# apache/parquet-mr

Measured on AMD Instinct MI355X. Metric: decoded values/s, device-resident int64 RLE_DICTIONARY pages, higher is better.
Workload: dtype int64; 1 GPU; C2: int64 RLE_DICTIONARY, 1k-cardinality dictionary (w=10), Zipf(a=1.5) run lengths in [1,4096], parquet-mr V1 pages of 20,000 values, uncompressed, one 100M-row row group per GPU; rows_per_gpu=100000000, pages_per_gpu=5000, encoded_data_bytes_per_gpu=4368634, parallelism=row-group shard x1

## Files before the change

### include/pqgpu.h

```cpp
#ifndef PQGPU_H
#define PQGPU_H

#include <stddef.h>
#include <stdint.h>

#ifdef __cplusplus
extern "C" {
#endif

#define PQG_ABI_VERSION 6

enum pqg_physical_type {
  PQG_BOOLEAN = 0,
  PQG_INT32 = 1,
  PQG_INT64 = 2,
  PQG_INT96 = 3,
  PQG_FLOAT = 4,
  PQG_DOUBLE = 5,
  PQG_BYTE_ARRAY = 6,
  PQG_FIXED_LEN_BYTE_ARRAY = 7
};

enum pqg_encoding {
  PQG_PLAIN = 0,
// ... 76 lines not shown
  int64_t value_index;
  char message[240];
} pqg_status;

typedef struct pqg_ctx pqg_ctx;
typedef struct pqg_plan pqg_plan;


int pqg_abi_version(void);

int pqg_device_count(void);

int pqg_ctx_create(int device, void* hip_stream, pqg_ctx** out);
int pqg_ctx_destroy(pqg_ctx* ctx);
void* pqg_ctx_stream(pqg_ctx* ctx);

enum pqg_dispatch {
  PQG_DISPATCH_PLAIN_ONE_PASS = 1,
  PQG_DISPATCH_DICT_DIRECT = 2,
  PQG_DISPATCH_GZIP_PREPASS_MIN = 3,
  PQG_DISPATCH_DICT_FUSED = 4,
  PQG_DISPATCH_NULL_HINTS = 5,
  PQG_DISPATCH_TAKE_STAGED = 6,
  PQG_DISPATCH_ZSTD_PREPASS = 7
};
int pqg_ctx_set_dispatch(pqg_ctx* ctx, int key, int value);

int pqg_decode(pqg_ctx* ctx, const uint8_t* d_bytes, uint64_t n_bytes,
               pqg_column_desc* cols, int n_cols,
               const pqg_page_desc* pages, int n_pages,
               uint32_t* d_page_value_counts, pqg_status* st);

int pqg_sync(pqg_ctx* ctx, pqg_status* st);

enum pqg_phase {
  PQG_PHASE_NONE = 0,
  PQG_PHASE_DICTIONARY = 1,
  PQG_PHASE_RL_INIT = 2,
  PQG_PHASE_DL_INIT = 3,
  PQG_PHASE_DATA_INIT = 4,
  PQG_PHASE_RL_READ = 5,
  PQG_PHASE_DL_READ = 6,
  PQG_PHASE_VALUE = 7
};

typedef struct pqg_page_error {
  int32_t code;
// ... 321 lines not shown
```

### parquet-mr_amd/csrc/pqgpu_api.hip

```cpp
#include <hip/hip_runtime.h>

#include <algorithm>
#include <chrono>
#include <cstdio>
#include <cstddef>
#include <cstdlib>
#include <cstring>
#include <new>
#include <atomic>
#include <thread>
#include <type_traits>
#include <vector>

#include "pqgpu_internal.h"
#include "pqgpu_filter.h"
#include "pqgpu_take.h"

using pqg::ColumnDev;
using pqg::PageWork;
using pqg::HostErr;
using pqg::bin_out;
using pqg::elem_width;
using pqg::out_width;
using pqg::C_DICT4; using pqg::C_DICT8; using pqg::C_IDS; using pqg::C_PLAIN; using pqg::C_BOOL; using pqg::C_DELTA4;
// ... 73 lines not shown
  bool zero;
};

template <class T>
PlanBufInit uploaded(PlanBuf b, const std::vector<T>& v, size_t min_elems) {
  return PlanBufInit{b, v.data(), sizeof(T) * v.size(), sizeof(T) * std::max(v.size(), min_elems), false};
}

}

struct pqg_plan {
  pqg_ctx* ctx = nullptr;
  const uint8_t* d_bytes = nullptr;
  uint64_t n_bytes = 0;
  pqg::PlanLayout L;
  DevBuf buf[B_COUNT];
  uint32_t* dba_meta() const {
    return L.dba_meta_off == pqg::NO_REGION ? nullptr : (uint32_t*)((uint8_t*)buf[B_BSCRATCH].p + L.dba_meta_off);
  }
  uint32_t epoch = 0;
  uint32_t err_epoch = pqg::ERR_EPOCH_MAX;
  uint32_t pseg_epoch = 0;
  bool dict_fused = true;
  bool plain_fused = false;
  bool seg_walk = true;
  bool null_hints = false;
  int kernels = 0;
  int timeout_fallbacks = 0;
  int plain_fallbacks = 0;
  int hint_fallbacks = 0;
  uint32_t* d_counts = nullptr;
  std::vector<pqg_page_error> page_errs;
};

struct RouterCache {
  int w = -1;
  uint64_t tail_len = 0;
  std::vector<uint8_t> bytes;
  std::vector<uint64_t> off;
  std::vector<uint32_t> cnt;
  std::vector<uint64_t> vo;
  std::vector<int32_t> vals;
  uint64_t hits = 0, misses = 0;
};

struct pqg_ctx {
// ... 6 lines not shown
  std::vector<pqg_staged_output> staged;
  pqg_column_desc* last_cols = nullptr;
  PinnedBuf pin_in, pin_out, pin_err;
  DevBuf host_bytes, host_out, host_counts, host_runs;
  DevBuf asm_scratch;
  hipStream_t copy_stream = nullptr;
  DevBuf zstd_scratch;
  DevBuf zstd_seqs, zstd_mode;
  DevBuf gzip_recs, gzip_mode;
  hipStream_t side_stream = nullptr;
  hipEvent_t ev_fork = nullptr, ev_join = nullptr;
  hipStream_t bin_stream = nullptr;
  hipEvent_t ev_join_bin = nullptr;
  hipStream_t fix_stream = nullptr;
  hipEvent_t ev_join_fix = nullptr;
  hipStream_t dent_stream = nullptr;
  hipEvent_t ev_dent_fork = nullptr, ev_dent = nullptr;
  int plain_mode = 2;
  bool dict_direct = true;
  bool dict_fused = true;
  bool null_hints = true;
  uint32_t gz_prepass_min = pqg::GZ_PREPASS_MIN;
  bool zstd_prepass = true;
  RouterCache router;
  DevBuf filter_scratch, filter_image;
  uint64_t filter_serial = 0;
  DevBuf filter_dict;
  PinnedBuf filter_dict_pin;
  hipEvent_t filter_dict_ev[4] = {};
  uint32_t filter_dict_seq = 0;
  pqg_column_desc dict_desc = {};
  pqg_column_desc* dict_user = nullptr;
  static constexpr int TAKE_SLOTS = 4;
  static constexpr size_t TAKE_SLOT_BYTES = sizeof(pqg::TakeRecDev) * pqg::TAKE_REC_MAX_RECORDS;
  DevBuf take_scratch, take_cols;
  PinnedBuf take_pin;
  hipEvent_t take_ev[TAKE_SLOTS] = {};
  uint32_t take_seq = 0;
  bool take_staged = true;
};

extern "C" {

int pqg_abi_version(void) { return PQG_ABI_VERSION; }

const char* pqg_error_name(int code) {
// ... 13 lines not shown
    case PQG_ERR_NO_DICTIONARY: return "NO_DICTIONARY";
    case PQG_ERR_DICT_ENCODING: return "DICT_ENCODING";
    case PQG_ERR_CRC: return "CRC";
    default: return "UNKNOWN";
  }
}

int pqg_device_count(void) {
  int n = 0;
  if (hipGetDeviceCount(&n) != hipSuccess) return 0;
  return n;
}

int pqg_ctx_create(int device, void* hip_stream, pqg_ctx** out) {
  if (!out) return PQG_ERR_INVALID_ARG;
  *out = nullptr;
  int n = pqg_device_count();
  if (n <= 0) return PQG_ERR_NO_DEVICE;
  if (device < 0 || device >= n) return PQG_ERR_INVALID_ARG;
  if (hipSetDevice(device) != hipSuccess) return PQG_ERR_HIP;
  pqg_ctx* c = new (std::nothrow) pqg_ctx();
  if (!c) return PQG_ERR_INVALID_ARG;
  c->device = device;
  if (hip_stream) {
    c->stream = (hipStream_t)hip_stream;
  } else {
    if (hipStreamCreateWithFlags(&c->stream, hipStreamNonBlocking) != hipSuccess) {
      delete c;
      return PQG_ERR_HIP;
    }
    c->own_stream = true;
  }
  if (hipStreamCreateWithFlags(&c->side_stream, hipStreamNonBlocking) != hipSuccess) c->side_stream = nullptr;
  if (hipStreamCreateWithFlags(&c->bin_stream, hipStreamNonBlocking) != hipSuccess) c->bin_stream = nullptr;
  if (hipStreamCreateWithFlags(&c->fix_stream, hipStreamNonBlocking) != hipSuccess) c->fix_stream = nullptr;
  *out = c;
  return PQG_OK;
}

void* pqg_ctx_stream(pqg_ctx* ctx) { return ctx ? (void*)ctx->stream : nullptr; }

int pqg_ctx_set_dispatch(pqg_ctx* ctx, int key, int value) {
  if (!ctx) return PQG_ERR_INVALID_ARG;
  switch (key) {
    case PQG_DISPATCH_PLAIN_ONE_PASS:
      if (value < 0 || value > 3) return PQG_ERR_INVALID_ARG;
// ... 2 lines not shown
    case PQG_DISPATCH_DICT_DIRECT:
      if (value != 0 && value != 1) return PQG_ERR_INVALID_ARG;
      ctx->dict_direct = value != 0;
      return PQG_OK;
    case PQG_DISPATCH_GZIP_PREPASS_MIN:
      if (value < 0) return PQG_ERR_INVALID_ARG;
      ctx->gz_prepass_min = (uint32_t)value;
      return PQG_OK;
    case PQG_DISPATCH_DICT_FUSED:
      if (value != 0 && value != 1) return PQG_ERR_INVALID_ARG;
      ctx->dict_fused = value != 0;
      return PQG_OK;
    case PQG_DISPATCH_NULL_HINTS:
      if (value != 0 && value != 1) return PQG_ERR_INVALID_ARG;
      ctx->null_hints = value != 0;
      return PQG_OK;
    case PQG_DISPATCH_TAKE_STAGED:
      if (value != 0 && value != 1) return PQG_ERR_INVALID_ARG;
      ctx->take_staged = value != 0;
      return PQG_OK;
    case PQG_DISPATCH_ZSTD_PREPASS:
      if (value != 0 && value != 1) return PQG_ERR_INVALID_ARG;
      ctx->zstd_prepass = value != 0;
      return PQG_OK;
    default: return PQG_ERR_INVALID_ARG;
  }
}

int pqg_plan_destroy(pqg_plan* p);

int pqg_ctx_destroy(pqg_ctx* c) {
  if (!c) return PQG_OK;
  (void)hipSetDevice(c->device);
  (void)hipStreamSynchronize(c->stream);
  if (c->last) pqg_plan_destroy(c->last);
  c->pin_in.release();
  c->pin_out.release();
  c->pin_err.release();
  c->host_bytes.release();
  c->host_out.release();
  c->host_counts.release();
  c->host_runs.release();
  c->asm_scratch.release();
  c->zstd_scratch.release();
  c->zstd_seqs.release();
  c->zstd_mode.release();
// ... 49 lines not shown
                            const pqg_column_desc* cols, int n_cols, const pqg_page_desc* pages, int n_pages,
                            pqg_plan** out, pqg_status* st) {
  if (st) { std::memset(st, 0, sizeof(*st)); st->page = -1; }
  if (!ctx || !out || n_cols < 0 || n_pages < 0 || (n_cols && !cols) || (n_pages && !pages) || (n_bytes && !d_bytes) ||
      ((uintptr_t)d_bytes & 3u)) {
    set_status(st, PQG_ERR_INVALID_ARG, -1, -1, "plan arguments");
    return PQG_ERR_INVALID_ARG;
  }
  if (hipSetDevice(ctx->device) != hipSuccess) return PQG_ERR_HIP;
  pqg_plan* P = new (std::nothrow) pqg_plan();
  if (!P) return PQG_ERR_INVALID_ARG;
  P->ctx = ctx;
  P->d_bytes = d_bytes;
  P->n_bytes = n_bytes;
  pqg::PlanLayout& L = P->L;
  int bad_page = -1;
  if (pqg::plan_layout(n_bytes, valid_bytes, cols, n_cols, pages, n_pages,
                       pqg::PlanOptions{ctx->plain_mode, ctx->dict_direct, ctx->null_hints}, &L, &bad_page) != PQG_OK) {
    set_status(st, PQG_ERR_INVALID_ARG, bad_page, -1, "page descriptor");
    delete P;
    return PQG_ERR_INVALID_ARG;
  }
  P->dict_fused = ctx->dict_fused;
  P->plain_fused = L.n_pcp != 0;
  P->null_hints = L.null_hints;
  const size_t pages1 = (size_t)std::max(n_pages, 1);
  const PlanBufInit init[B_COUNT] = {
      uploaded(B_WORK, L.h_work, 0),
      uploaded(B_COLS, L.cols, 0),
      uploaded(B_LISTS, L.flat, 1),
      uploaded(B_COL_PAGES, L.cp, 1),
      uploaded(B_COL_PAGE_START, L.cps, 0),
      {B_ERR, nullptr, 0, err_region_bytes(n_pages, n_cols) + 16, false},
      {B_BSCRATCH, nullptr, 0, (size_t)std::max<uint64_t>(L.scratch_bytes, 256), false},
      uploaded(B_BIN_LISTS, L.bl, 1),
      uploaded(B_BIN_BLOCKS, L.bin_blocks, 1),
      uploaded(B_BIN_CHUNKS, L.bin_chunks, 1),
      uploaded(B_DBA_CHUNKS, L.dba_chunks, 1),
      uploaded(B_SEGS, L.segs, 1),
      uploaded(B_DENT_TILES, L.dent_tiles, 1),
      uploaded(B_PSEGS, L.psegs, 1),
      {B_PSTATUS, nullptr, 2 * sizeof(uint64_t) * L.psegs.size(), 2 * sizeof(uint64_t) * std::max<size_t>(L.psegs.size(), 1), true},
      uploaded(B_PCOL_PAGES, L.pcp, 1),
      {B_PCOL_START, L.pcs.data(), L.pcp.empty() ? 0 : sizeof(int32_t) * L.pcs.size(), sizeof(int32_t) * L.pcs.size(), false},
      {B_REC, nullptr, 0, sizeof(uint64_t) * (size_t)(L.rec_total + 2 * 64 + 16), false},
      {B_CHUNK_RUN, nullptr, 0, sizeof(uint32_t) * std::max<uint32_t>(L.chunk_total, 1), false},
// ... 138 lines not shown
                           (uint32_t*)((uint8_t*)P->buf[B_BSCRATCH].p + P->L.hint_off));
  if (e == hipSuccess && pf) {
    uint8_t* scb = (uint8_t*)P->buf[B_BSCRATCH].p;
    uint64_t* ps = (uint64_t*)P->buf[B_PSTATUS].p;
    e = pqg::launch_bin_plain(fork ? ctx->side_stream : s, P->d_bytes, P->n_bytes, work, cols, (const int32_t*)P->buf[B_PCOL_PAGES].p,
                              (const int32_t*)P->buf[B_PCOL_START].p, P->L.n_pcols, (const uint64_t*)P->buf[B_PSEGS].p, P->L.n_psegs, ps,
                              ps + P->L.n_psegs, (uint32_t*)(scb + P->L.pticket_off), P->pseg_epoch,
                              (uint32_t*)(scb + P->L.pflag_off), P->err_epoch, err, ecount, P->L.plain_pg, P->L.n_pcp);
    if (fork && hipEventRecord(ctx->ev_join, ctx->side_stream) != hipSuccess) e = hipErrorUnknown;
  }
  const hipStream_t sb = fork_bin ? ctx->bin_stream : s;
  const hipStream_t sf = fork_fix ? ctx->fix_stream : s;
  if (e == hipSuccess) e = launch_dict_walks(sb);
  for (int k = 0; k < C_NCLS && e == hipSuccess; k++) {
    int n = P->L.cls_n[k] - (k == C_BINP ? P->L.n_binp_seg + (pf ? P->L.n_binp_fused : 0) : 0);
    if (!n) continue;
    const int32_t* l = lists + P->L.cls_off[k];
    switch (k) {
      case C_DICT4:
      case C_DICT8: {
        const int i = k - C_DICT4;
        e = pqg::launch_dict(k == C_DICT8 ? 8 : 4, sf, P->d_bytes, P->n_bytes, work, cols, l, n, (uint64_t*)P->buf[B_REC].p,
                             (uint32_t*)P->buf[B_CHUNK_RUN].p, (const uint64_t*)P->buf[B_CHUNKS].p + P->L.chunk_off[i], P->L.chunk_n[i],
                             (uint64_t*)P->buf[B_PSTAT].p, (uint32_t*)P->buf[B_FLAGS].p, P->epoch, P->dict_fused, err, ecount);
        break;
      }
      case C_IDS: {
        const int i = k - C_DICT4;
        e = pqg::launch_dict_ids(sb, P->d_bytes, P->n_bytes, work, cols, l, n, (uint64_t*)P->buf[B_REC].p,
                                 (uint32_t*)P->buf[B_CHUNK_RUN].p, (const uint64_t*)P->buf[B_CHUNKS].p + P->L.chunk_off[i],
                                 P->L.chunk_n[i], (uint64_t*)P->buf[B_PSTAT].p, (uint32_t*)P->buf[B_FLAGS].p, P->epoch, P->dict_fused, err, ecount);
        break;
      }
      case C_DD:
      case C_DDG: {
        const int g = k == C_DDG ? 1 : 0;
        e = pqg::launch_dict_dd(sb, P->d_bytes, P->n_bytes, work, cols, l, n, (uint64_t*)P->buf[B_REC].p,
                                (uint32_t*)P->buf[B_CHUNK_RUN].p, (const uint64_t*)P->buf[B_CHUNKS].p + P->L.dd_chunk_off[g],
                                P->L.dd_chunk_n[g], (uint64_t*)P->buf[B_PSTAT].p, (uint32_t*)P->buf[B_FLAGS].p, P->epoch, P->dict_fused,
                                err, ecount, (uint64_t*)((uint8_t*)P->buf[B_BSCRATCH].p + P->L.dd_sums_off[g]),
                                bl + P->L.off_dd_cols[g], bl + P->L.off_dd_start[g], P->L.n_dd_cols[g], P->L.dd_region, g == 1,
                                g == 1 && dent_fork ? ctx->ev_dent : nullptr);
        break;
      }
      case C_BSS: e = pqg::launch_bss(sf, P->d_bytes, P->n_bytes, work, cols, l, n, err, ecount); break;
      case C_BINP:
        e = pqg::launch_bin_walk(sb, P->d_bytes, P->n_bytes, work, cols, l, n, 0, P->L.n_pages, err, ecount);
        break;
      case C_DLBA: e = pqg::launch_dlba_lengths(sb, P->d_bytes, P->n_bytes, work, cols, l, n, err, ecount); break;
      case C_DBA:
        e = pqg::launch_dba_lengths(sb, P->d_bytes, P->n_bytes, work, cols, l, n, err, ecount, P->dba_meta());
        break;
      case C_PLAIN: e = pqg::launch_plain(0, sf, P->d_bytes, P->n_bytes, work, cols, l, n, err, ecount); break;
      case C_BOOL: e = pqg::launch_plain(1, sf, P->d_bytes, P->n_bytes, work, cols, l, n, err, ecount); break;
      case C_RLEBOOL: e = pqg::launch_plain(2, sf, P->d_bytes, P->n_bytes, work, cols, l, n, err, ecount); break;
      case C_DELTA4: e = pqg::launch_delta(4, sf, P->d_bytes, P->n_bytes, work, cols, l, n, err, ecount); break;
      case C_DELTA8: e = pqg::launch_delta(8, sf, P->d_bytes, P->n_bytes, work, cols, l, n, err, ecount); break;
    }
  }
  if (e == hipSuccess && P->L.n_segs && !P->seg_walk)
    e = pqg::launch_bin_walk(sb, P->d_bytes, P->n_bytes, work, cols,
                             lists + P->L.cls_off[C_BINP] + (P->L.cls_n[C_BINP] - P->L.n_binp_seg), P->L.n_binp_seg, 0,
                             P->L.n_pages, err, ecount);
// ... 1369 lines not shown
```

### parquet-mr_amd/csrc/pqgpu_internal.h

```cpp
#pragma once
#include <hip/hip_runtime.h>
#include <stdint.h>

#include "../../include/pqgpu.h"
#include "pqgpu_filter.h"
#include "pqgpu_plan.h"

namespace pqg {

struct ErrCount {
  uint32_t* p;
  uint32_t epoch;
};
constexpr uint32_t ERR_EPOCH_MAX = 0xFFFFu;
constexpr uint64_t ERR_KEY_MASK = (1ull << 48) - 1;

hipError_t launch_dict(int width, hipStream_t st, const uint8_t* bytes, uint64_t n_bytes, PageWork* work,
                       const ColumnDev* cols, const int32_t* list, int n, uint64_t* rec, uint32_t* chunk_run,
                       const uint64_t* chunks, uint32_t n_chunks, uint64_t* pstat, uint32_t* flags, uint32_t epoch,
                       bool fused, uint64_t* err,
                       ErrCount err_count);
hipError_t launch_levels(hipStream_t st, const uint8_t* bytes, uint64_t n_bytes, PageWork* work, const ColumnDev* cols,
                         const int32_t* list, int n, uint64_t* err, ErrCount err_count, uint32_t* hint_bad);
hipError_t launch_scan(hipStream_t st, PageWork* work, const int32_t* col_pages, const int32_t* col_page_start,
                       int n_cols);
hipError_t launch_plain(int kind, hipStream_t st, const uint8_t* bytes, uint64_t n_bytes, PageWork* work,
                        const ColumnDev* cols, const int32_t* list, int n, uint64_t* err, ErrCount err_count);
hipError_t launch_delta(int width, hipStream_t st, const uint8_t* bytes, uint64_t n_bytes, PageWork* work,
                        const ColumnDev* cols, const int32_t* list, int n, uint64_t* err, ErrCount err_count);
hipError_t launch_dict_ids(hipStream_t st, const uint8_t* bytes, uint64_t n_bytes, PageWork* work,
                           const ColumnDev* cols, const int32_t* list, int n, uint64_t* rec, uint32_t* chunk_run,
                           const uint64_t* chunks, uint32_t n_chunks, uint64_t* pstat, uint32_t* flags,
                           uint32_t epoch, bool fused,
                           uint64_t* err, ErrCount err_count);
hipError_t launch_dict_dd(hipStream_t st, const uint8_t* bytes, uint64_t n_bytes, PageWork* work,
                          const ColumnDev* cols, const int32_t* list, int n, uint64_t* rec, uint32_t* chunk_run,
                          const uint64_t* chunks, uint32_t n_chunks, uint64_t* pstat, uint32_t* flags,
                          uint32_t epoch, bool fused, uint64_t* err, ErrCount err_count, uint64_t* sums,
                          const int32_t* dd_cols, const int32_t* dd_start, int n_dd_cols, uint32_t dd_region,
                          bool global, hipEvent_t entries_ready = nullptr);
hipError_t launch_dlba_lengths(hipStream_t st, const uint8_t* bytes, uint64_t n_bytes, PageWork* work,
                               const ColumnDev* cols, const int32_t* list, int n, uint64_t* err, ErrCount err_count);
constexpr uint64_t ZSTD_LIT_SCRATCH = 131072;
constexpr uint32_t ZSTD_GRID = 4096;
hipError_t launch_zstd(hipStream_t st, const uint8_t* src, uint64_t src_bytes, uint8_t* dst, uint64_t dst_bytes,
                       const pqg_snappy_job* jobs, int n_jobs, int32_t* status, uint8_t* scratch, uint64_t* seqs,
                       int32_t* mode);
hipError_t launch_snappy(hipStream_t st, const uint8_t* src, uint64_t src_bytes, uint8_t* dst, uint64_t dst_bytes,
                         const void* jobs, int n_jobs, int32_t* status);
hipError_t launch_lz4raw(hipStream_t st, const uint8_t* src, uint64_t src_bytes, uint8_t* dst, uint64_t dst_bytes,
                         const void* jobs, int n_jobs, int32_t* status);
constexpr uint32_t GZ_PREPASS_MIN = 16384;
hipError_t launch_gzip(hipStream_t st, const uint8_t* src, uint64_t src_bytes, uint8_t* dst, uint64_t dst_bytes,
                       const void* jobs, int n_jobs, int32_t* status, uint64_t* recs, int32_t* mode,
                       uint32_t prepass_min = GZ_PREPASS_MIN);
constexpr uint32_t DBA_VB = 2048;
hipError_t launch_dba_lengths(hipStream_t st, const uint8_t* bytes, uint64_t n_bytes, PageWork* work,
                              const ColumnDev* cols, const int32_t* list, int n, uint64_t* err, ErrCount err_count,
                              uint32_t* dba_meta);
hipError_t launch_dba_copy(hipStream_t st, const uint8_t* bytes, uint64_t n_bytes, PageWork* work,
                           const ColumnDev* cols, const int32_t* list, int n, const uint64_t* chunks,
                           uint32_t n_chunks, const uint32_t* dba_meta, const int32_t* carry_cols, int n_carry_cols,
// ... 75 lines not shown
```

### parquet-mr_amd/csrc/pqgpu_kernels.hip

```cpp
#include <hip/hip_runtime.h>
#include <stdint.h>

#include <type_traits>

#include "pqgpu_device.h"

namespace pqg {


struct PreWin {
  rsrc_t rs;
  uint8_t* seg;
  uint32_t seg_lo;
  uint32_t B;
  uint32_t nxt[4];
  uint32_t cnt[4];
  uint32_t val[4];
  uint32_t flg;
};

constexpr uint32_t SEG_BYTES = 3072;


__device__ __forceinline__ void seg_fill(PreWin& pw, uint32_t lo) {
// ... 903 lines not shown
  __shared__ __attribute__((aligned(16))) uint8_t lds[XT_LDS_BYTES];
  dict_tiles_body<W, false, IDS>(bytes, n_bytes, work, cols, rec, chunk_run, chunks, n_chunks, pstat, nullptr, 0,
                                 err, err_count, lds, blockIdx.x);
}

template <int W, bool IDS = false>
__global__ __launch_bounds__(64 * WPB) void k_dict_fused(const uint8_t* __restrict__ bytes, uint64_t n_bytes,
                                                         const PageWork* __restrict__ work,
                                                         const ColumnDev* __restrict__ cols,
                                                         const int32_t* __restrict__ list, int n_list,
                                                         uint32_t n_walk, uint64_t* rec, uint32_t* chunk_run,
                                                         const uint64_t* __restrict__ chunks, uint32_t n_chunks,
                                                         uint64_t* pstat, uint32_t* flags, uint32_t epoch,
                                                         uint64_t* err, ErrCount err_count) {
  constexpr uint32_t LB = sizeof(DictWaveLds) * WPB > XT_LDS_BYTES ? sizeof(DictWaveLds) * WPB : XT_LDS_BYTES;
  __shared__ __attribute__((aligned(16))) uint8_t lds[LB];
  if (blockIdx.x < n_walk) {
#ifdef PQG_FAULT_INJECT
    if (blockIdx.x == 0) {
      const uint64_t t0 = __builtin_amdgcn_s_memrealtime();
      while (__builtin_amdgcn_s_memrealtime() - t0 < (uint64_t)PQG_FAULT_INJECT) __builtin_amdgcn_s_sleep(127);
    }
#endif
    dict_runs_body<W>(bytes, n_bytes, work, cols, list, n_list, rec, chunk_run, pstat, flags, epoch, err, err_count,
                      lds, blockIdx.x);
  } else {
    dict_tiles_body<W, true, IDS>(bytes, n_bytes, work, cols, rec, chunk_run, chunks, n_chunks, pstat, flags, epoch,
                                  err, err_count, lds, blockIdx.x - n_walk);
  }
}


template <int DDM>
__global__ __launch_bounds__(64 * WPB) void k_dict_fused_dd(const uint8_t* __restrict__ bytes, uint64_t n_bytes,
                                                            const PageWork* __restrict__ work,
                                                            const ColumnDev* __restrict__ cols,
                                                            const int32_t* __restrict__ list, int n_list,
                                                            uint32_t n_walk, uint64_t* rec, uint32_t* chunk_run,
                                                            const uint64_t* __restrict__ chunks, uint32_t n_chunks,
                                                            uint64_t* pstat, uint32_t* flags, uint32_t epoch,
                                                            uint64_t* err, ErrCount err_count, uint64_t* sums) {
  constexpr uint32_t LB = sizeof(DictWaveLds) * WPB > XT_LDS_BYTES ? sizeof(DictWaveLds) * WPB : XT_LDS_BYTES;
  __shared__ __attribute__((aligned(16))) uint8_t lds[LB];
  if (blockIdx.x < n_walk) {
#ifdef PQG_FAULT_INJECT
    if (blockIdx.x == 0) {
      const uint64_t t0 = __builtin_amdgcn_s_memrealtime();
      while (__builtin_amdgcn_s_memrealtime() - t0 < (uint64_t)PQG_FAULT_INJECT) __builtin_amdgcn_s_sleep(127);
    }
#endif
    dict_runs_body<4>(bytes, n_bytes, work, cols, list, n_list, rec, chunk_run, pstat, flags, epoch, err, err_count,
                      lds, blockIdx.x);
  } else {
    dict_tiles_body<4, true, true, DDM>(bytes, n_bytes, work, cols, rec, chunk_run, chunks, n_chunks, pstat, flags,
                                        epoch, err, err_count, lds, blockIdx.x - n_walk, sums);
  }
}

template <int DDM>
__global__ __launch_bounds__(64 * WPB) void k_dict_tiles_dd(const uint8_t* __restrict__ bytes, uint64_t n_bytes,
                                                            const PageWork* __restrict__ work,
                                                            const ColumnDev* __restrict__ cols, const uint64_t* rec,
                                                            const uint32_t* chunk_run,
                                                            const uint64_t* __restrict__ chunks, uint32_t n_chunks,
                                                            const uint64_t* pstat, uint64_t* err, ErrCount err_count,
                                                            uint64_t* sums) {
  __shared__ __attribute__((aligned(16))) uint8_t lds[XT_LDS_BYTES];
  dict_tiles_body<4, false, true, DDM>(bytes, n_bytes, work, cols, rec, chunk_run, chunks, n_chunks, pstat,
                                       nullptr, 0, err, err_count, lds, blockIdx.x, sums);
}

constexpr uint32_t DDB_PER = 16;
__global__ __launch_bounds__(256) void k_dd_bases(const PageWork* __restrict__ work, const ColumnDev* __restrict__ cols,
                                                  const uint64_t* __restrict__ chunks, const int32_t* __restrict__ dd_cols,
                                                  const int32_t* __restrict__ start, uint64_t* sums) {
// ... 2259 lines not shown
  return hipMemcpyToSymbol(HIP_SYMBOL(pqg::pqg_diag_nostore), &v, sizeof(v)) == hipSuccess ? 0 : 3;
}
extern "C" int pqg_diag_set(void* p) {
  return hipMemcpyToSymbol(HIP_SYMBOL(pqg::pqg_diag_buf), &p, sizeof(p)) == hipSuccess ? 0 : 3;
}
extern "C" int pqg_diag_wph_set(void* p) {
  return hipMemcpyToSymbol(HIP_SYMBOL(pqg::pqg_diag_wph), &p, sizeof(p)) == hipSuccess ? 0 : 3;
}
extern "C" int pqg_diag_rt_set(void* walk, void* chunk) {
  return hipMemcpyToSymbol(HIP_SYMBOL(pqg::pqg_diag_wrt), &walk, sizeof(walk)) == hipSuccess &&
                 hipMemcpyToSymbol(HIP_SYMBOL(pqg::pqg_diag_xrt), &chunk, sizeof(chunk)) == hipSuccess
             ? 0
             : 3;
}
namespace pqg {
#endif


#define PQG_LAUNCH_ARGS bytes, n_bytes, work, cols, list, n, err, err_count

hipError_t launch_dict(int width, hipStream_t st, const uint8_t* bytes, uint64_t n_bytes, PageWork* work,
                       const ColumnDev* cols, const int32_t* list, int n, uint64_t* rec, uint32_t* chunk_run,
                       const uint64_t* chunks, uint32_t n_chunks, uint64_t* pstat, uint32_t* flags, uint32_t epoch,
                       bool fused, uint64_t* err, ErrCount err_count) {
  if (n <= 0) return hipSuccess;
  const uint32_t n_walk = (uint32_t)(n + WPB - 1) / WPB, n_tile = (n_chunks + WPB - 1) / WPB;
  const dim3 blk(64 * WPB);
  if (fused) {
    if (width == 8)
      hipLaunchKernelGGL(k_dict_fused<8>, dim3(n_walk + n_tile), blk, 0, st, bytes, n_bytes, work, cols, list, n, n_walk,
                         rec, chunk_run, chunks, n_chunks, pstat, flags, epoch, err, err_count);
    else
      hipLaunchKernelGGL(k_dict_fused<4>, dim3(n_walk + n_tile), blk, 0, st, bytes, n_bytes, work, cols, list, n, n_walk,
                         rec, chunk_run, chunks, n_chunks, pstat, flags, epoch, err, err_count);
    return hipGetLastError();
  }
  if (width == 8) {
    hipLaunchKernelGGL(k_dict_runs<8>, dim3(n_walk), blk, 0, st, bytes, n_bytes, work, cols, list, n, rec, chunk_run,
                       pstat, flags, epoch, err, err_count);
    if (n_tile)
      hipLaunchKernelGGL(k_dict_tiles<8>, dim3(n_tile), blk, 0, st, bytes, n_bytes, work, cols, rec, chunk_run, chunks,
                         n_chunks, pstat, err, err_count);
  } else {
    hipLaunchKernelGGL(k_dict_runs<4>, dim3(n_walk), blk, 0, st, bytes, n_bytes, work, cols, list, n, rec, chunk_run,
                       pstat, flags, epoch, err, err_count);
    if (n_tile)
      hipLaunchKernelGGL(k_dict_tiles<4>, dim3(n_tile), blk, 0, st, bytes, n_bytes, work, cols, rec, chunk_run, chunks,
                         n_chunks, pstat, err, err_count);
  }
  return hipGetLastError();
}

hipError_t launch_dict_ids(hipStream_t st, const uint8_t* bytes, uint64_t n_bytes, PageWork* work,
                           const ColumnDev* cols, const int32_t* list, int n, uint64_t* rec, uint32_t* chunk_run,
                           const uint64_t* chunks, uint32_t n_chunks, uint64_t* pstat, uint32_t* flags,
                           uint32_t epoch, bool fused, uint64_t* err, ErrCount err_count) {
  if (n <= 0) return hipSuccess;
  const uint32_t n_walk = (uint32_t)(n + WPB - 1) / WPB, n_tile = (n_chunks + WPB - 1) / WPB;
  const dim3 blk(64 * WPB);
  if (fused) {
    hipLaunchKernelGGL((k_dict_fused<4, true>), dim3(n_walk + n_tile), blk, 0, st, bytes, n_bytes, work, cols, list, n,
                       n_walk, rec, chunk_run, chunks, n_chunks, pstat, flags, epoch, err, err_count);
    return hipGetLastError();
  }
  hipLaunchKernelGGL(k_dict_runs<4>, dim3(n_walk), blk, 0, st, bytes, n_bytes, work, cols, list, n, rec, chunk_run,
                     pstat, flags, epoch, err, err_count);
  if (n_tile)
    hipLaunchKernelGGL((k_dict_tiles<4, true>), dim3(n_tile), blk, 0, st, bytes, n_bytes, work, cols, rec, chunk_run,
                       chunks, n_chunks, pstat, err, err_count);
  return hipGetLastError();
}

hipError_t launch_dict_dd(hipStream_t st, const uint8_t* bytes, uint64_t n_bytes, PageWork* work,
                          const ColumnDev* cols, const int32_t* list, int n, uint64_t* rec, uint32_t* chunk_run,
                          const uint64_t* chunks, uint32_t n_chunks, uint64_t* pstat, uint32_t* flags,
                          uint32_t epoch, bool fused, uint64_t* err, ErrCount err_count, uint64_t* sums,
                          const int32_t* dd_cols, const int32_t* dd_start, int n_dd_cols, uint32_t dd_region,
                          bool global, hipEvent_t entries_ready) {
  if (n <= 0) return hipSuccess;
  const uint32_t n_walk = (uint32_t)(n + WPB - 1) / WPB, n_tile = (n_chunks + WPB - 1) / WPB;
  const dim3 blk(64 * WPB);
  if (fused) {
    if (global)
      hipLaunchKernelGGL(k_dict_fused_dd<DD_IDS>, dim3(n_walk + n_tile), blk, 0, st, bytes, n_bytes, work, cols, list, n,
                         n_walk, rec, chunk_run, chunks, n_chunks, pstat, flags, epoch, err, err_count, sums);
    else
      hipLaunchKernelGGL(k_dict_fused_dd<DD_SUMS>, dim3(n_walk + n_tile), blk, 0, st, bytes, n_bytes, work, cols, list, n,
                         n_walk, rec, chunk_run, chunks, n_chunks, pstat, flags, epoch, err, err_count, sums);
  } else {
    hipLaunchKernelGGL(k_dict_runs<4>, dim3(n_walk), blk, 0, st, bytes, n_bytes, work, cols, list, n, rec, chunk_run,
                       pstat, flags, epoch, err, err_count);
    if (n_tile) {
      if (global)
        hipLaunchKernelGGL(k_dict_tiles_dd<DD_IDS>, dim3(n_tile), blk, 0, st, bytes, n_bytes, work, cols, rec, chunk_run,
                           chunks, n_chunks, pstat, err, err_count, sums);
      else
        hipLaunchKernelGGL(k_dict_tiles_dd<DD_SUMS>, dim3(n_tile), blk, 0, st, bytes, n_bytes, work, cols, rec, chunk_run,
                           chunks, n_chunks, pstat, err, err_count, sums);
    }
  }
  hipError_t e = hipGetLastError();
  if (e != hipSuccess) return e;
  if (entries_ready && hipStreamWaitEvent(st, entries_ready, 0) != hipSuccess) return hipErrorUnknown;
  if (global && n_tile) {
    hipLaunchKernelGGL(k_dd_gsums, dim3(n_tile), blk, 0, st, work, cols, chunks, n_chunks, pstat, sums);
    e = hipGetLastError();
    if (e != hipSuccess) return e;
  }
  hipLaunchKernelGGL(k_dd_bases, dim3(n_dd_cols), dim3(256), 0, st, work, cols, chunks, dd_cols, dd_start, sums);
  e = hipGetLastError();
  if (e != hipSuccess || !n_tile) return e;
// ... 75 lines not shown
```

### parquet-mr_amd/csrc/pqgpu_plan.h

```cpp
#pragma once
#include <stdint.h>

#include <vector>

#include "../../include/pqgpu.h"

namespace pqg {

struct ColumnDev {
  int32_t physical_type;
  int32_t type_length;
  int32_t max_rep;
  int32_t max_def;
  int32_t elem_width;
  uint32_t dict_n;
  uint64_t dict_offset;
  uint64_t dict_bytes;
  void* values;
  uint8_t* def_levels;
  uint8_t* rep_levels;
  uint8_t* binary_data;
  uint64_t binary_capacity;
  uint32_t* blen;
  uint32_t* bsrc;
// ... 136 lines not shown
  uint64_t seg_status_off = 0, seg_tmp_off = 0;
  bool plain_pg = false;
  int n_pcp = 0;
  uint32_t n_psegs = 0;
  int n_pcols = 0;
  uint64_t pticket_off = 0, pflag_off = 0;
  int n_binp_fused = 0, n_bin_cols_nf = 0;
  int n_binp_seg = 0;
  uint32_t n_bin_blocks_nf = 0, n_bin_chunks_nf = 0;
  bool null_hints = false;
  uint64_t hint_off = 0;
  std::vector<int> page_cls;
  std::vector<uint8_t> col_nullable;
  std::vector<uint64_t> col_required_values;
  std::vector<int> col_first_page;
  std::vector<uint64_t> bin_capacity;
  std::vector<void*> empty_bin_values;
  std::vector<HostErr> host_errs;
};

int plan_layout(uint64_t n_bytes, uint64_t valid_bytes, const pqg_column_desc* cols, int n_cols,
                const pqg_page_desc* pages, int n_pages, const PlanOptions& opt, PlanLayout* out, int* bad_page);

int plan_kernel_count(const PlanLayout& L, bool plain_fused, bool dict_fused, bool null_hints);

}
```

### parquet-mr_amd/csrc/pqgpu_plan_host.cpp

```cpp
#include "pqgpu_plan.h"

#include <algorithm>
#include <cstring>

namespace pqg {

namespace {

struct Planner {
  const uint64_t valid_bytes;
  const pqg_column_desc* const cols;
  const int n_cols;
  const pqg_page_desc* const pages;
  const int n_pages;
  const PlanOptions opt;
  PlanLayout& L;

  const size_t nc, np;
  std::vector<int> col_err;
  std::vector<std::vector<int>> cls_lists;
  std::vector<int> lvl_list;
  std::vector<std::vector<int>> col_pages;
  std::vector<std::vector<int>> col_all_pages;
  std::vector<uint64_t> slot_acc, val_acc;
// ... 521 lines not shown
  P.dba_chunks();
  P.dict_chunks();
  P.scratch_regions();
  P.flatten_lists();
  return PQG_OK;
}

int plan_kernel_count(const PlanLayout& L, bool plain_fused, bool dict_fused, bool null_hints) {
  const bool pf = plain_fused;
  int k = (L.levels_n ? 1 : 0) + (L.n_scan_cols && !null_hints ? 1 : 0);
  for (int c = 0; c < C_NCLS; c++) {
    const int n = L.cls_n[c] - (c == C_BINP ? L.n_binp_seg + (pf ? L.n_binp_fused : 0) : 0);
    if (n && c == C_DD) k += dict_fused ? 3 : 4;
    else if (n && c == C_DDG) k += dict_fused ? 4 : 5;
    else if (n) k += (c == C_DICT4 || c == C_DICT8 || c == C_IDS) && !dict_fused ? 2 : 1;
  }
  k += (L.n_dict_walk ? 1 : 0) + (L.n_dent_tiles ? 3 : 0) + (L.n_bind ? 1 : 0) + (L.n_fixd ? 1 : 0) +
       ((pf ? L.n_bin_blocks_nf : L.n_bin_blocks) ? 3 : 0) + ((pf ? L.n_bin_chunks_nf : L.n_bin_chunks) ? 1 : 0) +
       (L.cls_n[C_DBA] ? (L.n_dba_chunks ? 4 : 1) : 0) + (L.n_carry ? 1 : 0) + (L.n_segs ? 1 : 0) +
       (pf ? 2 : 0);
  return k;
}

}
```

### parquet-mr_amd/pqgpu/abi.py

```python
import ctypes as C

import numpy as np

ABI_VERSION = 6

BOOLEAN, INT32, INT64, INT96, FLOAT, DOUBLE, BYTE_ARRAY, FIXED_LEN_BYTE_ARRAY = range(8)
TYPE_NAMES = {BOOLEAN: "BOOLEAN", INT32: "INT32", INT64: "INT64", INT96: "INT96", FLOAT: "FLOAT",
              DOUBLE: "DOUBLE", BYTE_ARRAY: "BYTE_ARRAY", FIXED_LEN_BYTE_ARRAY: "FIXED_LEN_BYTE_ARRAY"}

PLAIN = 0
PLAIN_DICTIONARY = 2
RLE = 3
BIT_PACKED = 4
DELTA_BINARY_PACKED = 5
DELTA_LENGTH_BYTE_ARRAY = 6
DELTA_BYTE_ARRAY = 7
RLE_DICTIONARY = 8
BYTE_STREAM_SPLIT = 9

OK = 0
ERR_INVALID_ARG = 1
ERR_UNSUPPORTED = 2
ERR_HIP = 3
ERR_NO_DEVICE = 4
# ... 155 lines not shown

def numpy_dtype(physical_type, type_length=0):
    if physical_type == BOOLEAN:
        return np.dtype(np.uint8)
    if physical_type == INT32:
        return np.dtype("<i4")
    if physical_type == INT64:
        return np.dtype("<i8")
    if physical_type == FLOAT:
        return np.dtype("<f4")
    if physical_type == DOUBLE:
        return np.dtype("<f8")
    if physical_type == BYTE_ARRAY:
        return np.dtype("<i8")
    return np.dtype((np.void, elem_width(physical_type, type_length)))

DISPATCH_PLAIN_ONE_PASS = 1
DISPATCH_DICT_DIRECT = 2
DISPATCH_GZIP_PREPASS_MIN = 3
DISPATCH_DICT_FUSED = 4
DISPATCH_TAKE_STAGED = 6
DISPATCH_ZSTD_PREPASS = 7
DISPATCH_NULL_HINTS = 5


FILTER_TILE_ROWS = 4096
FILTER_MAX_NODES = 64
FILTER_MAX_LITERALS = 4096
FILTER_MAX_LITERAL_BYTES = 16384
(FILTER_EQ, FILTER_NOTEQ, FILTER_LT, FILTER_LTEQ, FILTER_GT, FILTER_GTEQ, FILTER_IN, FILTER_NOTIN, FILTER_AND,
 FILTER_OR, FILTER_NOT, FILTER_CONTAINS) = range(12)
FILTER_NULL_LITERAL = 1
FILTER_UNSIGNED = 2


class FilterNode(C.Structure):
    _fields_ = [("op", C.c_int32), ("column", C.c_int32), ("left", C.c_int32), ("right", C.c_int32),
                ("flags", C.c_uint32), ("literal_begin", C.c_uint32), ("n_literals", C.c_uint32),
                ("reserved", C.c_uint32)]


class FilterColumn(C.Structure):
    _fields_ = [("physical_type", C.c_int32), ("max_def", C.c_int32), ("values", C.c_void_p),
                ("binary_data", C.c_void_p), ("def_levels", C.c_void_p), ("n_values", C.c_uint64)]


# ... 68 lines not shown
```

Baseline: 565.0 billion values/s.

## Cap dictionary run-walker blocks with a cost model and grid-stride persistent walkers

Fused dictionary kernels now launch a limited number of persistent walker blocks that grid-stride over the page groups, instead of one block per group. The host estimates how many walkers to use from a per-page walk-cost model and an output-store bandwidth model, with the CU count as a floor and an override available through a new dispatch key. The aim is to free CU slots for the tile-expansion blocks that share the grid, so walking and storing overlap better. The risk is that too few walkers lengthen the critical path when walking dominates, and the cost constants are tuned by hand.

```diff
diff --git a/include/pqgpu.h b/include/pqgpu.h
--- a/include/pqgpu.h
+++ b/include/pqgpu.h
@@ -122,7 +122,8 @@
   PQG_DISPATCH_DICT_FUSED = 4,
   PQG_DISPATCH_NULL_HINTS = 5,
   PQG_DISPATCH_TAKE_STAGED = 6,
-  PQG_DISPATCH_ZSTD_PREPASS = 7
+  PQG_DISPATCH_ZSTD_PREPASS = 7,
+  PQG_DISPATCH_DICT_WALKERS = 8
 };
 int pqg_ctx_set_dispatch(pqg_ctx* ctx, int key, int value);
 
diff --git a/parquet-mr_amd/csrc/pqgpu_api.hip b/parquet-mr_amd/csrc/pqgpu_api.hip
--- a/parquet-mr_amd/csrc/pqgpu_api.hip
+++ b/parquet-mr_amd/csrc/pqgpu_api.hip
@@ -119,6 +119,7 @@
   uint32_t err_epoch = pqg::ERR_EPOCH_MAX;
   uint32_t pseg_epoch = 0;
   bool dict_fused = true;
+  uint32_t walk_groups[pqg::C_NCLS] = {};
   bool plain_fused = false;
   bool seg_walk = true;
   bool null_hints = false;
@@ -171,6 +172,8 @@
   bool null_hints = true;
   uint32_t gz_prepass_min = pqg::GZ_PREPASS_MIN;
   bool zstd_prepass = true;
+  int dict_walkers = 0x7fffffff;
+  int n_cus = 256;
   RouterCache router;
   DevBuf filter_scratch, filter_image;
   uint64_t filter_serial = 0;
@@ -230,6 +233,8 @@
   pqg_ctx* c = new (std::nothrow) pqg_ctx();
   if (!c) return PQG_ERR_INVALID_ARG;
   c->device = device;
+  int cus = 0;
+  if (hipDeviceGetAttribute(&cus, hipDeviceAttributeMultiprocessorCount, device) == hipSuccess && cus > 0) c->n_cus = cus;
   if (hip_stream) {
     c->stream = (hipStream_t)hip_stream;
   } else {
@@ -278,6 +283,10 @@
     case PQG_DISPATCH_ZSTD_PREPASS:
       if (value != 0 && value != 1) return PQG_ERR_INVALID_ARG;
       ctx->zstd_prepass = value != 0;
+      return PQG_OK;
+    case PQG_DISPATCH_DICT_WALKERS:
+      if (value < 0) return PQG_ERR_INVALID_ARG;
+      ctx->dict_walkers = value;
       return PQG_OK;
     default: return PQG_ERR_INVALID_ARG;
   }
@@ -373,6 +382,10 @@
     return PQG_ERR_INVALID_ARG;
   }
   P->dict_fused = ctx->dict_fused;
+  for (int k : {(int)C_DICT4, (int)C_DICT8, (int)C_IDS, (int)C_DD, (int)C_DDG}) {
+    const int ew = k == C_DICT8 ? 8 : k == C_DD || k == C_DDG ? 2 : 4;
+    P->walk_groups[k] = pqg::dict_walk_groups(L, L.flat.data() + L.cls_off[k], L.cls_n[k], ew, ctx->n_cus, ctx->dict_walkers);
+  }
   P->plain_fused = L.n_pcp != 0;
   P->null_hints = L.null_hints;
   const size_t pages1 = (size_t)std::max(n_pages, 1);
@@ -557,14 +570,14 @@
         const int i = k - C_DICT4;
         e = pqg::launch_dict(k == C_DICT8 ? 8 : 4, sf, P->d_bytes, P->n_bytes, work, cols, l, n, (uint64_t*)P->buf[B_REC].p,
                              (uint32_t*)P->buf[B_CHUNK_RUN].p, (const uint64_t*)P->buf[B_CHUNKS].p + P->L.chunk_off[i], P->L.chunk_n[i],
-                             (uint64_t*)P->buf[B_PSTAT].p, (uint32_t*)P->buf[B_FLAGS].p, P->epoch, P->dict_fused, err, ecount);
+                             (uint64_t*)P->buf[B_PSTAT].p, (uint32_t*)P->buf[B_FLAGS].p, P->epoch, P->dict_fused, P->walk_groups[k], err, ecount);
         break;
       }
       case C_IDS: {
         const int i = k - C_DICT4;
         e = pqg::launch_dict_ids(sb, P->d_bytes, P->n_bytes, work, cols, l, n, (uint64_t*)P->buf[B_REC].p,
                                  (uint32_t*)P->buf[B_CHUNK_RUN].p, (const uint64_t*)P->buf[B_CHUNKS].p + P->L.chunk_off[i],
-                                 P->L.chunk_n[i], (uint64_t*)P->buf[B_PSTAT].p, (uint32_t*)P->buf[B_FLAGS].p, P->epoch, P->dict_fused, err, ecount);
+                                 P->L.chunk_n[i], (uint64_t*)P->buf[B_PSTAT].p, (uint32_t*)P->buf[B_FLAGS].p, P->epoch, P->dict_fused, P->walk_groups[k], err, ecount);
         break;
       }
       case C_DD:
@@ -573,7 +586,7 @@
         e = pqg::launch_dict_dd(sb, P->d_bytes, P->n_bytes, work, cols, l, n, (uint64_t*)P->buf[B_REC].p,
                                 (uint32_t*)P->buf[B_CHUNK_RUN].p, (const uint64_t*)P->buf[B_CHUNKS].p + P->L.dd_chunk_off[g],
                                 P->L.dd_chunk_n[g], (uint64_t*)P->buf[B_PSTAT].p, (uint32_t*)P->buf[B_FLAGS].p, P->epoch, P->dict_fused,
-                                err, ecount, (uint64_t*)((uint8_t*)P->buf[B_BSCRATCH].p + P->L.dd_sums_off[g]),
+                                P->walk_groups[k], err, ecount, (uint64_t*)((uint8_t*)P->buf[B_BSCRATCH].p + P->L.dd_sums_off[g]),
                                 bl + P->L.off_dd_cols[g], bl + P->L.off_dd_start[g], P->L.n_dd_cols[g], P->L.dd_region, g == 1,
                                 g == 1 && dent_fork ? ctx->ev_dent : nullptr);
         break;
diff --git a/parquet-mr_amd/csrc/pqgpu_internal.h b/parquet-mr_amd/csrc/pqgpu_internal.h
--- a/parquet-mr_amd/csrc/pqgpu_internal.h
+++ b/parquet-mr_amd/csrc/pqgpu_internal.h
@@ -18,7 +18,7 @@
 hipError_t launch_dict(int width, hipStream_t st, const uint8_t* bytes, uint64_t n_bytes, PageWork* work,
                        const ColumnDev* cols, const int32_t* list, int n, uint64_t* rec, uint32_t* chunk_run,
                        const uint64_t* chunks, uint32_t n_chunks, uint64_t* pstat, uint32_t* flags, uint32_t epoch,
-                       bool fused, uint64_t* err,
+                       bool fused, uint32_t walk_groups, uint64_t* err,
                        ErrCount err_count);
 hipError_t launch_levels(hipStream_t st, const uint8_t* bytes, uint64_t n_bytes, PageWork* work, const ColumnDev* cols,
                          const int32_t* list, int n, uint64_t* err, ErrCount err_count, uint32_t* hint_bad);
@@ -31,13 +31,13 @@
 hipError_t launch_dict_ids(hipStream_t st, const uint8_t* bytes, uint64_t n_bytes, PageWork* work,
                            const ColumnDev* cols, const int32_t* list, int n, uint64_t* rec, uint32_t* chunk_run,
                            const uint64_t* chunks, uint32_t n_chunks, uint64_t* pstat, uint32_t* flags,
-                           uint32_t epoch, bool fused,
+                           uint32_t epoch, bool fused, uint32_t walk_groups,
                            uint64_t* err, ErrCount err_count);
 hipError_t launch_dict_dd(hipStream_t st, const uint8_t* bytes, uint64_t n_bytes, PageWork* work,
                           const ColumnDev* cols, const int32_t* list, int n, uint64_t* rec, uint32_t* chunk_run,
                           const uint64_t* chunks, uint32_t n_chunks, uint64_t* pstat, uint32_t* flags,
-                          uint32_t epoch, bool fused, uint64_t* err, ErrCount err_count, uint64_t* sums,
-                          const int32_t* dd_cols, const int32_t* dd_start, int n_dd_cols, uint32_t dd_region,
+                          uint32_t epoch, bool fused, uint32_t walk_groups, uint64_t* err, ErrCount err_count,
+                          uint64_t* sums, const int32_t* dd_cols, const int32_t* dd_start, int n_dd_cols, uint32_t dd_region,
                           bool global, hipEvent_t entries_ready = nullptr);
 hipError_t launch_dlba_lengths(hipStream_t st, const uint8_t* bytes, uint64_t n_bytes, PageWork* work,
                                const ColumnDev* cols, const int32_t* list, int n, uint64_t* err, ErrCount err_count);
diff --git a/parquet-mr_amd/csrc/pqgpu_kernels.hip b/parquet-mr_amd/csrc/pqgpu_kernels.hip
--- a/parquet-mr_amd/csrc/pqgpu_kernels.hip
+++ b/parquet-mr_amd/csrc/pqgpu_kernels.hip
@@ -949,8 +949,11 @@
       while (__builtin_amdgcn_s_memrealtime() - t0 < (uint64_t)PQG_FAULT_INJECT) __builtin_amdgcn_s_sleep(127);
     }
 #endif
-    dict_runs_body<W>(bytes, n_bytes, work, cols, list, n_list, rec, chunk_run, pstat, flags, epoch, err, err_count,
-                      lds, blockIdx.x);
+    for (uint32_t g = blockIdx.x; g < ((uint32_t)n_list + WPB - 1u) / WPB; g += n_walk) {
+      dict_runs_body<W>(bytes, n_bytes, work, cols, list, n_list, rec, chunk_run, pstat, flags, epoch, err, err_count,
+                        lds, g);
+      wave_sync();
+    }
   } else {
     dict_tiles_body<W, true, IDS>(bytes, n_bytes, work, cols, rec, chunk_run, chunks, n_chunks, pstat, flags, epoch,
                                   err, err_count, lds, blockIdx.x - n_walk);
@@ -976,8 +979,11 @@
       while (__builtin_amdgcn_s_memrealtime() - t0 < (uint64_t)PQG_FAULT_INJECT) __builtin_amdgcn_s_sleep(127);
     }
 #endif
-    dict_runs_body<4>(bytes, n_bytes, work, cols, list, n_list, rec, chunk_run, pstat, flags, epoch, err, err_count,
-                      lds, blockIdx.x);
+    for (uint32_t g = blockIdx.x; g < ((uint32_t)n_list + WPB - 1u) / WPB; g += n_walk) {
+      dict_runs_body<4>(bytes, n_bytes, work, cols, list, n_list, rec, chunk_run, pstat, flags, epoch, err, err_count,
+                        lds, g);
+      wave_sync();
+    }
   } else {
     dict_tiles_body<4, true, true, DDM>(bytes, n_bytes, work, cols, rec, chunk_run, chunks, n_chunks, pstat, flags,
                                         epoch, err, err_count, lds, blockIdx.x - n_walk, sums);
@@ -3283,16 +3289,17 @@
 hipError_t launch_dict(int width, hipStream_t st, const uint8_t* bytes, uint64_t n_bytes, PageWork* work,
                        const ColumnDev* cols, const int32_t* list, int n, uint64_t* rec, uint32_t* chunk_run,
                        const uint64_t* chunks, uint32_t n_chunks, uint64_t* pstat, uint32_t* flags, uint32_t epoch,
-                       bool fused, uint64_t* err, ErrCount err_count) {
+                       bool fused, uint32_t walk_groups, uint64_t* err, ErrCount err_count) {
   if (n <= 0) return hipSuccess;
   const uint32_t n_walk = (uint32_t)(n + WPB - 1) / WPB, n_tile = (n_chunks + WPB - 1) / WPB;
+  const uint32_t n_pers = walk_groups && walk_groups < n_walk ? walk_groups : n_walk;
   const dim3 blk(64 * WPB);
   if (fused) {
     if (width == 8)
-      hipLaunchKernelGGL(k_dict_fused<8>, dim3(n_walk + n_tile), blk, 0, st, bytes, n_bytes, work, cols, list, n, n_walk,
+      hipLaunchKernelGGL(k_dict_fused<8>, dim3(n_pers + n_tile), blk, 0, st, bytes, n_bytes, work, cols, list, n, n_pers,
                          rec, chunk_run, chunks, n_chunks, pstat, flags, epoch, err, err_count);
     else
-      hipLaunchKernelGGL(k_dict_fused<4>, dim3(n_walk + n_tile), blk, 0, st, bytes, n_bytes, work, cols, list, n, n_walk,
+      hipLaunchKernelGGL(k_dict_fused<4>, dim3(n_pers + n_tile), blk, 0, st, bytes, n_bytes, work, cols, list, n, n_pers,
                          rec, chunk_run, chunks, n_chunks, pstat, flags, epoch, err, err_count);
     return hipGetLastError();
   }
@@ -3315,13 +3322,14 @@
 hipError_t launch_dict_ids(hipStream_t st, const uint8_t* bytes, uint64_t n_bytes, PageWork* work,
                            const ColumnDev* cols, const int32_t* list, int n, uint64_t* rec, uint32_t* chunk_run,
                            const uint64_t* chunks, uint32_t n_chunks, uint64_t* pstat, uint32_t* flags,
-                           uint32_t epoch, bool fused, uint64_t* err, ErrCount err_count) {
+                           uint32_t epoch, bool fused, uint32_t walk_groups, uint64_t* err, ErrCount err_count) {
   if (n <= 0) return hipSuccess;
   const uint32_t n_walk = (uint32_t)(n + WPB - 1) / WPB, n_tile = (n_chunks + WPB - 1) / WPB;
+  const uint32_t n_pers = walk_groups && walk_groups < n_walk ? walk_groups : n_walk;
   const dim3 blk(64 * WPB);
   if (fused) {
-    hipLaunchKernelGGL((k_dict_fused<4, true>), dim3(n_walk + n_tile), blk, 0, st, bytes, n_bytes, work, cols, list, n,
-                       n_walk, rec, chunk_run, chunks, n_chunks, pstat, flags, epoch, err, err_count);
+    hipLaunchKernelGGL((k_dict_fused<4, true>), dim3(n_pers + n_tile), blk, 0, st, bytes, n_bytes, work, cols, list, n,
+                       n_pers, rec, chunk_run, chunks, n_chunks, pstat, flags, epoch, err, err_count);
     return hipGetLastError();
   }
   hipLaunchKernelGGL(k_dict_runs<4>, dim3(n_walk), blk, 0, st, bytes, n_bytes, work, cols, list, n, rec, chunk_run,
@@ -3335,19 +3343,20 @@
 hipError_t launch_dict_dd(hipStream_t st, const uint8_t* bytes, uint64_t n_bytes, PageWork* work,
                           const ColumnDev* cols, const int32_t* list, int n, uint64_t* rec, uint32_t* chunk_run,
                           const uint64_t* chunks, uint32_t n_chunks, uint64_t* pstat, uint32_t* flags,
-                          uint32_t epoch, bool fused, uint64_t* err, ErrCount err_count, uint64_t* sums,
-                          const int32_t* dd_cols, const int32_t* dd_start, int n_dd_cols, uint32_t dd_region,
+                          uint32_t epoch, bool fused, uint32_t walk_groups, uint64_t* err, ErrCount err_count,
+                          uint64_t* sums, const int32_t* dd_cols, const int32_t* dd_start, int n_dd_cols, uint32_t dd_region,
                           bool global, hipEvent_t entries_ready) {
   if (n <= 0) return hipSuccess;
   const uint32_t n_walk = (uint32_t)(n + WPB - 1) / WPB, n_tile = (n_chunks + WPB - 1) / WPB;
+  const uint32_t n_pers = walk_groups && walk_groups < n_walk ? walk_groups : n_walk;
   const dim3 blk(64 * WPB);
   if (fused) {
     if (global)
-      hipLaunchKernelGGL(k_dict_fused_dd<DD_IDS>, dim3(n_walk + n_tile), blk, 0, st, bytes, n_bytes, work, cols, list, n,
-                         n_walk, rec, chunk_run, chunks, n_chunks, pstat, flags, epoch, err, err_count, sums);
+      hipLaunchKernelGGL(k_dict_fused_dd<DD_IDS>, dim3(n_pers + n_tile), blk, 0, st, bytes, n_bytes, work, cols, list, n,
+                         n_pers, rec, chunk_run, chunks, n_chunks, pstat, flags, epoch, err, err_count, sums);
     else
-      hipLaunchKernelGGL(k_dict_fused_dd<DD_SUMS>, dim3(n_walk + n_tile), blk, 0, st, bytes, n_bytes, work, cols, list, n,
-                         n_walk, rec, chunk_run, chunks, n_chunks, pstat, flags, epoch, err, err_count, sums);
+      hipLaunchKernelGGL(k_dict_fused_dd<DD_SUMS>, dim3(n_pers + n_tile), blk, 0, st, bytes, n_bytes, work, cols, list, n,
+                         n_pers, rec, chunk_run, chunks, n_chunks, pstat, flags, epoch, err, err_count, sums);
   } else {
     hipLaunchKernelGGL(k_dict_runs<4>, dim3(n_walk), blk, 0, st, bytes, n_bytes, work, cols, list, n, rec, chunk_run,
                        pstat, flags, epoch, err, err_count);
diff --git a/parquet-mr_amd/csrc/pqgpu_plan.h b/parquet-mr_amd/csrc/pqgpu_plan.h
--- a/parquet-mr_amd/csrc/pqgpu_plan.h
+++ b/parquet-mr_amd/csrc/pqgpu_plan.h
@@ -182,6 +182,8 @@
 int plan_layout(uint64_t n_bytes, uint64_t valid_bytes, const pqg_column_desc* cols, int n_cols,
                 const pqg_page_desc* pages, int n_pages, const PlanOptions& opt, PlanLayout* out, int* bad_page);
 
+uint32_t dict_walk_groups(const PlanLayout& L, const int32_t* list, int n, int elem_width, int n_cus, int override_groups);
+
 int plan_kernel_count(const PlanLayout& L, bool plain_fused, bool dict_fused, bool null_hints);
 
 }
diff --git a/parquet-mr_amd/csrc/pqgpu_plan_host.cpp b/parquet-mr_amd/csrc/pqgpu_plan_host.cpp
--- a/parquet-mr_amd/csrc/pqgpu_plan_host.cpp
+++ b/parquet-mr_amd/csrc/pqgpu_plan_host.cpp
@@ -567,4 +567,35 @@
   return k;
 }
 
+namespace {
+constexpr double WALK_A_US = 5.2;
+constexpr double WALK_B_US = 2.68;
+constexpr double STORE_BYTES_PER_US = 5.2e6;
+constexpr double WALK_LEAD = 2.0;
 }
+
+uint32_t dict_walk_groups(const PlanLayout& L, const int32_t* list, int n, int elem_width, int n_cus, int override_groups) {
+  if (n <= 0 || !list) return 0;
+  const uint32_t full = ((uint32_t)n + (uint32_t)DICT_WPB - 1) / (uint32_t)DICT_WPB;
+  if (override_groups > 0) return std::min<uint32_t>((uint32_t)override_groups, full);
+  double cost_us = 0, out_bytes = 0;
+  for (int i = 0; i < n; i++) {
+    const int p = list[i];
+    if (p < 0 || (size_t)p >= L.h_work.size()) continue;
+    const PageWork& w = L.h_work[(size_t)p];
+    const bool known = w.column >= 0 && (size_t)w.column < L.col_nullable.size() &&
+                       (!L.col_nullable[(size_t)w.column] || L.null_hints);
+    const uint32_t sec = known && w.data_begin <= w.size ? w.size - w.data_begin : w.size;
+    cost_us += WALK_A_US + WALK_B_US * (double)((sec + 255u) / 256u);
+    out_bytes += (double)w.num_slots * (double)std::max(elem_width, 1);
+  }
+  const uint32_t lo = std::min<uint32_t>(full, (uint32_t)std::max(n_cus, 1));
+  const double store_us = out_bytes / STORE_BYTES_PER_US;
+  if (!(store_us > 0)) return full;
+  const double waves = WALK_LEAD * cost_us / store_us;
+  if (!(waves < (double)full * DICT_WPB)) return full;
+  const uint32_t groups = ((uint32_t)waves + (uint32_t)DICT_WPB) / (uint32_t)DICT_WPB;
+  return std::min(full, std::max(lo, groups));
+}
+
+}
diff --git a/parquet-mr_amd/pqgpu/abi.py b/parquet-mr_amd/pqgpu/abi.py
--- a/parquet-mr_amd/pqgpu/abi.py
+++ b/parquet-mr_amd/pqgpu/abi.py
@@ -201,6 +201,7 @@
 DISPATCH_TAKE_STAGED = 6
 DISPATCH_ZSTD_PREPASS = 7
 DISPATCH_NULL_HINTS = 5
+DISPATCH_DICT_WALKERS = 8
 
 
 FILTER_TILE_ROWS = 4096
```

After: 559.9 billion values/s. About the same (-0.9%).
